# marinlauber/WaterLily

Hardware: AMD Instinct MI355X
Metric: MLUPS (cell-updates/s) per sim_step!, 3D sphere (higher is better)
Workload: dtype f32; 1 GPU; 3D sphere 512x512x512, Re=3700, f32, uniform inflow, remeasure=false (BASELINE configs[2]); layout=padded, transport=none, comm_ranks=1, scalar_allreduce=none

## Files before the change

profiles/parse_pmc.py:

```python
#!/usr/bin/env python3
import collections
import csv
import json
import os
import re
import sys

LAMBDA = {
    ("op_pcg", "k_range_red", "#1"): "pcg_init", ("op_pcg", "k_range_red", "#2"): "pcg_mult_dot",
    ("op_pcg", "k_range_red", "#3"): "pcg_update", ("op_pcg", "k_range", "#1"): "pcg_direction",
    ("op_increment", "k_range", "#1"): "increment", ("op_jacobi", "k_range", "#1"): "jacobi",
    ("op_residual", "k_range_red", "#1"): "residual", ("op_bdim2", "k_range", "#1"): "bdim",
    ("op_correct", "k_range", "#1"): "correct", ("op_div", "k_range", "#1"): "div",
}


S7 = {"op_pcg": "pcg_mult_dot", "op_increment": "increment", "op_residual": "residual", "op_smooth_fused": "smooth",
      "op_prolong_increment_fused": "prolongate"}


ROWVEC = {("op_pcg", "#1"): "pcg_init", ("op_pcg", "#2"): "pcg_update", ("op_pcg", "#3"): "pcg_direction",
          ("op_bdim2", "#1"): "bdim", ("op_scale_all", "#1"): "scale"}


def classify(name):
    if "k_convdiff3" in name:
        return "conv_diff"
    if "k_correct3" in name:
        return "correct"
    if "k_measure_fill" in name:
        return "measure_fill"
    if "k_measure_rows" in name:
        return "measure_rows"
    if "k_scale_flat" in name:
        return "scale"
    if "k_rowvec" in name:
        m = re.search(r"(op_\w+?)<", name)
        o = re.search(r"#(\d)\}", name)
        return ROWVEC.get((m.group(1), "#" + o.group(1))) if m and o else None
    if "k_stencil7" in name:
        if "ResidualDivEpi" in name:
            return "residual"
        m = re.search(r"(op_\w+?)<", name)
        return S7.get(m.group(1)) if m else None
    m = re.search(r"(k_range_red|k_range)<.*?(op_\w+?)<", name)
    o = re.search(r"#(\d)\}", name)
    if not m or not o:
        return None
    return LAMBDA.get((m.group(2), m.group(1), "#" + o.group(1)))


def collect(path, counter):
    per = collections.defaultdict(list)
    for r in csv.DictReader(open(path)):
        if r["Counter_Name"] != counter:
            continue
        k = classify(r["Kernel_Name"])
        if k:
            per[k].append(float(r["Counter_Value"]) * 1024.0)
    out, info = {}, {}
    for k, v in per.items():
        top = max(v)
        fin = [x for x in v if x > 0.25 * top]
        out[k] = sum(fin) / len(fin)
        info[k] = (len(fin), min(fin), max(fin))
    return out, info


def csrc_digest():
    import hashlib
    root = os.path.dirname(os.path.dirname(os.path.abspath(__file__)))
    h = hashlib.sha1()
    d = os.path.join(root, "waterlily_amd", "csrc")
    for f in sorted(os.listdir(d)) + [os.path.join("..", "..", "include", "wlhip.h")]:
        p = os.path.join(d, f)
# ... 34 lines not shown
```

profiles/summarize_trace.py:

```python
#!/usr/bin/env python3
import collections
import csv
import re
import sys


def short(n):
    if "k_convdiff3" in n:
        return "conv_diff(lds)"
    if "ResidualDivEpi" in n:
        rr = re.search(r"k_stencil7<\w+, \d, (\d)", n)
        return f"op_residual+div[stencil7{',R=' + rr.group(1) if rr else ''}]"
    m = re.search(r"(k_stencil7|k_rowvec|k_range_red|k_range|k_finalize|k_reduce_only|k_apply)<.*?(op_\w+?|red_\w+?)<", n)
    if m:
        lam = re.search(r"#(\d)\}", n)
        rr = re.search(r"k_stencil7<\w+, \d, (\d)", n)
        return f"{m.group(2)}{'#' + lam.group(1) if lam else ''}[{m.group(1)[2:]}{',R=' + rr.group(1) if rr else ''}]"
    if "k_pforce" in n:
        return "pforce"
    return re.sub(r"<.*", "", n)[:40]


def main():
    path = sys.argv[1]
    steps = float(sys.argv[2]) if len(sys.argv) > 2 else 1.0
    durs = collections.defaultdict(list)
    for r in csv.DictReader(open(path)):
        durs[short(r["Kernel_Name"])].append((int(r["End_Timestamp"]) - int(r["Start_Timestamp"])) / 1e3)
    rows = []
    for k, v in durs.items():
        top = max(v)
        fin = [d for d in v if top >= 60 and d > 0.25 * top]
        rest = [d for d in v if not (top >= 60 and d > 0.25 * top)]
        rows.append((k, fin, rest))
    tot_f = sum(sum(f) for _, f, _ in rows)
    tot_r = sum(sum(r) for _, _, r in rows)
    print(f"{'kernel':52s} {'finest#':>8s} {'ms':>9s} {'avg us':>8s} {'min':>7s} {'max':>7s} | {'other#':>7s} {'ms':>8s} {'avg us':>7s}   (per {steps:g} step(s))")
    for k, f, r in sorted(rows, key=lambda x: -(sum(x[1]) + sum(x[2]))):
        fa = f"{sum(f) / len(f):8.1f} {min(f):7.1f} {max(f):7.1f}" if f else f"{'':8s} {'':7s} {'':7s}"
        ra = f"{sum(r) / len(r):7.1f}" if r else f"{'':7s}"
        print(f"{k:52s} {len(f) / steps:8.1f} {sum(f) / 1e3 / steps:9.3f} {fa} | {len(r) / steps:7.1f} {sum(r) / 1e3 / steps:8.3f} {ra}")
    print(f"{'TOTAL':52s} {'':8s} {tot_f / 1e3 / steps:9.3f} {'':24s} | {'':7s} {tot_r / 1e3 / steps:8.3f}")


if __name__ == "__main__":
# ... 2 lines not shown
```

waterlily_amd/csrc/wl_api.hip:

```cpp
#include <cstdarg>
#include <cstring>
#include <memory>

#include <fcntl.h>
#include <sys/mman.h>
#include <sys/stat.h>
#include <unistd.h>

#include <rccl/rccl.h>

#include "wl_ops.h"
#include "wl_coarse.h"
#include "wl_measure.h"
#include "wl_mesh.h"
#include "wl_stats.h"
#include "wl_probe.h"
#include "wl_integrals.h"
#include "wl_surface.h"
#include "wl_iso.h"
#include "wl_render.h"

namespace wl {

struct RcclComm : Comm {
// ... 223 lines not shown
    long nband = -1;
};

template <class T> static LevelT<T> lvl(const wl_mg *m, int l) {
    const wl_level_desc &d = m->lev[l];
    LevelT<T> o;
    o.g = mkG(&d.g);
    o.L = (T *)d.L; o.D = (T *)d.D; o.iD = (T *)d.iD; o.x = (T *)d.x; o.eps = (T *)d.eps; o.r = (T *)d.r; o.z = (T *)d.z;
    o.rowc = (opt(WL_OPT_ROW_CONST_L) && l < (int)m->rowc.size()) ? (const T *)m->rowc[l].get() : nullptr;
    return o;
}

template <class T, int D> static int mg_update(wl_mg *m, const unsigned char *dirty = nullptr) {
    {
        LevelT<T> p = lvl<T>(m, 0);
        WL_TRY((op_set_diag<T, D>(p.g, p.D, p.iD, p.L, dirty)));
        WL_TRY((halo_exchange<T>(p.g, p.iD, 1, 1)));
        if (D == 3 && m->rowc[0].get()) WL_TRY((op_lrow<T>(p.g, p.L, p.iD, (T *)m->rowc[0].get(), dirty)));
    }
    for (int l = 1; l < m->nlev; ++l) {
        LevelT<T> a = lvl<T>(m, l), b = lvl<T>(m, l - 1);
        WL_TRY((op_restrictL<T, D>(a.g, a.L, b.g, b.L, m->permask)));
        WL_TRY((coarse_L_finish<T, D>(a.g, a.L, b.g, m->permask)));
        WL_TRY((op_set_diag<T, D>(a.g, a.D, a.iD, a.L)));
        WL_TRY((halo_exchange<T>(a.g, a.iD, 1, 1)));
        if (D == 3 && m->rowc[l].get()) WL_TRY((op_lrow<T>(a.g, a.L, a.iD, (T *)m->rowc[l].get())));
    }
    return 0;
}

template <class T, int D> static int mg_vcycle(wl_mg *m, int l, int *pcg_np = nullptr) {
    LevelT<T> fine = lvl<T>(m, l), coarse = lvl<T>(m, l + 1);
    const bool fused = (m->permask == 0) && opt(WL_OPT_SMOOTH_FUSED);
    if (fused) WL_TRY((op_smooth_fused<T, D>(fine, fine.eps)));
    else WL_TRY((op_jacobi<T, D>(fine, 1, m->permask)));
    const bool zero_in_restrict = (m->permask == 0) && !coarse.g.dist && !fine.g.dist;
    WL_TRY((op_restrict<T, D>(coarse.g, coarse.r, fine.g, fused ? fine.eps : fine.r, zero_in_restrict ? coarse.x : (T *)nullptr)));
    if (ctx().comm && ctx().comm->size > 1 && fine.g.dist && !coarse.g.dist) {
        const int nzl = (fine.g.nzg - 2) / ctx().comm->size / 2;
        WL_TRY(ctx().comm->allgather(coarse.r + coarse.g.s[2], (size_t)nzl * coarse.g.s[2] * sizeof(T)));
    }
    if (!zero_in_restrict) {
        Prof p(WL_K_MISC, coarse.g.cells());
        WL_HIP(hipMemsetAsync(coarse.x, 0, (size_t)span(coarse.g) * sizeof(T), ctx().stream));
    }
    const long tail_cells = coarse_tail_cells();
    bool tail = tail_cells && fused && !coarse.g.dist && coarse.g.interior_cells() <= tail_cells && (m->nlev - (l + 1)) <= CV_MAXLEV;
    if (tail) {
        CoarseArgs<T> ca;
        ca.nlev = m->nlev - (l + 1);
        for (int q = 0; q < ca.nlev; ++q) {
            ca.lev[q] = lvl<T>(m, l + 1 + q);
            if (ca.lev[q].g.dist) tail = false;
        }
        if (tail) {
            Prof p(WL_K_SMOOTH, coarse.g.cells());
            if (opt(WL_OPT_COARSE_PCG_RESIDENT)) hipLaunchKernelGGL((k_coarse_vcycle<T, D, true>), dim3(1), dim3(CV_THREADS), 0, ctx().stream, ca);
            else hipLaunchKernelGGL((k_coarse_vcycle<T, D, false>), dim3(1), dim3(CV_THREADS), 0, ctx().stream, ca);
            WL_HIP(hipGetLastError());
        }
    }
    if (!tail) {
        int pre = -1;
        if (l + 2 < m->nlev) WL_TRY((mg_vcycle<T, D>(m, l + 1, pcg_np ? &pre : nullptr)));
        WL_TRY((op_pcg<T, D>(coarse, 6, m->permask, m->sc.partials.get(), m->sc.st.get(), false, pre)));
    }
    if (pcg_np) *pcg_np = -1;
    if (fused) return op_prolong_increment_fused<T, D>(fine, fine.eps, coarse.g, coarse.x, m->sc.partials.get(), pcg_np);
    WL_TRY((op_prolongate<T, D>(fine.g, fine.eps, coarse.g, coarse.x)));
    return op_increment<T, D>(fine, m->permask);
}

template <class T, int D> static int mg_Linf(wl_mg *m, int l) {
    LevelT<T> p = lvl<T>(m, l);
    const T *r = p.r;
    return op_reduce<T, D>(p.g, WL_K_DOT, RED_MAX, 0.0, [=] __device__(long I) { const double v = (double)r[I]; return v < 0 ? -v : v; },
                           m->sc.partials.get(), m->sc.st.get(), 1, true);
}
template <class T, int D> static int mg_log_row(wl_mg *m, int n, bool have_r2) {
    if (!have_r2) WL_TRY((op_L2<T, D>(lvl<T>(m, 0), m->sc.partials.get(), m->sc.st.get(), false)));
    WL_TRY((mg_Linf<T, D>(m, 0)));
    WL_TRY(m->sc.fetch());
    m->log.push_back((double)n); m->log.push_back(m->sc.hst.get()->out[1]); m->log.push_back(m->sc.hst.get()->r2);
    return 0;
}
template <class T, int D> static int mg_solve(wl_mg *m, double tol, int itmx, int *n_iter, const T *divu = nullptr, const G *gu = nullptr,
                                              bool halo_begun = false) {
    LevelT<T> p = lvl<T>(m, 0);
    WL_TRY((op_residual<T, D>(p, m->permask, m->sc.partials.get(), m->sc.st.get(), divu, gu, halo_begun)));
    int n = 0;
    if (m->log_on) WL_TRY((mg_log_row<T, D>(m, 0, false)));
    while (n < itmx) {
        int pre = -1;
        if (m->nlev > 1) WL_TRY((mg_vcycle<T, D>(m, 0, &pre)));
        WL_TRY((op_pcg<T, D>(p, 6, m->permask, m->sc.partials.get(), m->sc.st.get(), true, pre, true)));
        WL_TRY((op_L2<T, D>(p, m->sc.partials.get(), m->sc.st.get(), true)));
        WL_TRY(m->sc.fetch());
        ++n;
        const double r2 = m->sc.hst.get()->r2;
        if (m->log_on) WL_TRY((mg_log_row<T, D>(m, n, true)));
        if (r2 < tol) break;
// ... 22 lines not shown
    bool begun = false;
    if (fused_div && g.dist) {
        if (!head_done) WL_TRY((op_scale_all<T, D>(g, p.x, dts, false, dbl)));
        if (exchange_u) { WL_TRY((halo_begin2<T>(g, uv, D, 1, p.g, p.x, 1, 1))); begun = true; }
    } else if (exchange_u && D == 3 && g.dist && overlap_on() && R.hi[2] - R.lo[2] + 1 >= 2) {
        WL_TRY((halo_begin<T>(g, uv, D, 1)));
        int rc = head_done ? 0 : op_scale_all<T, D>(g, p.x, dts, false, dbl);
        if (!rc) rc = op_div<T, D>(g, p.z, (const T *)uv, R.lo[2], R.hi[2] - 1);
        WL_TRY(halo_end());
        if (rc) return rc;
        WL_TRY((op_div<T, D>(g, p.z, (const T *)uv, R.hi[2], R.hi[2])));
    } else {
        if (exchange_u) WL_TRY((halo_exchange<T>(g, uv, D, 1)));
        if (!fused_div) WL_TRY((op_div<T, D>(g, p.z, (const T *)uv)));
        if (!head_done) WL_TRY((op_scale_all<T, D>(g, p.x, dts, false, dbl)));
    }
    WL_TRY((mg_solve<T, D>(b, 1e-4, 32, n_iter, fused_div ? (const T *)uv : nullptr, &g, begun)));
    WL_TRY((op_correct<T, D>(g, uv, p.L, p.x, p.rowc, xbc, xdone)));
    return op_scale_all<T, D>(g, p.x, dts, true, dbl, tail_then);
}

template <class T, int D>
static int flow_mom_step(wl_flow *a, wl_mg *b, double dt, const double *U, const double *gp, const double *gc,
                         double *dt_next, int *n2) {
    const wl_flow_desc &d = a->d;
    const G g = mkG(&d.g);
    T *u = (T *)d.u, *u0 = (T *)d.u0, *f = (T *)d.f, *V = (T *)d.V, *mu0 = (T *)d.mu0, *mu1 = (T *)d.mu1;
    const XBc<T> xbc{(D == 3 && d.perdir_mask == 0 && opt(WL_OPT_BC_FUSED) && opt(WL_OPT_XGHOST_IN_KERNEL)) ? 1 : 0, d.exitBC ? 1 : 0, (T)U[0]};
    bool xd = false;
    bool turns = false;
    if constexpr (D == 3)
        turns = opt(WL_OPT_BDIM_IN_CONVDIFF) && opt(WL_OPT_BDIM_ROWFLAGS) && a->rowfree && a->busy.get() && d.perdir_mask == 0 && !d.exitBC && conv_diff_tiled<D>(g, 0);
    T *const up = turns ? u0 : u;
    const CdFin<T> fin1{up, a->rowfree, xbc.on, (T)U[0]}, fin2{u, a->rowfree, xbc.on, (T)U[0]};
    (void)fin1; (void)fin2;
    if (turns) {
        if constexpr (D == 3) {
            WL_TRY((op_conv_diff<T, D, true, false, 1>(g, f, u, d.nu, 0, u, V, dt, gp, gp != nullptr, nullptr, false, &fin1)));
            WL_TRY((op_bdim2_busy<T, 1>(g, up, up, f, V, mu0, mu1, a->busy.get(), a->nbusy, a->nbusy_lo, a->nbusy_hi, xbc, a->segfree())));
            xd = xbc.on != 0;
        }
    } else {
        WL_TRY((op_conv_diff<T, D, true, true>(g, f, u, d.nu, d.perdir_mask, nullptr, V, dt, gp, gp != nullptr, u0)));
        if (d.perdir_mask != 0) WL_TRY((op_sigma_ghosts<T, D>(g, (T *)d.sigma, u, d.nu, d.perdir_mask)));
        WL_TRY((op_bdim2<T, D, 1>(g, u, f, V, mu0, mu1, a->rowfree, a->busy.get(), a->nbusy, true, &xbc, &xd, a->segfree())));
    }
    WL_TRY((op_bc_vec<T, D>(g, up, U, d.exitBC, d.perdir_mask, xd)));
    if (d.exitBC) WL_TRY((op_exit_bc<T, D>(g, up, u0, U, dt, a->sc.partials.get(), a->sc.st.get())));
    const ScaleOp corr_head = project_scale<T>(dt, 0.5);
    const bool chain = opt(WL_OPT_SCALE_CHAIN) != 0;
    WL_TRY((flow_project<T, D>(a, b, dt, 1.0, &n2[0], true, false, chain ? &corr_head : nullptr, &xbc, &xd, up)));
    WL_TRY((op_bc_vec<T, D>(g, up, U, d.exitBC, d.perdir_mask, xd)));
    if (turns) {
        if constexpr (D == 3) {
            WL_TRY((op_conv_diff<T, D, true, false, 2>(g, f, up, d.nu, 0, u, V, dt, gc, gc != nullptr, nullptr, true, &fin2)));
            WL_TRY((op_sigma_ghosts<T, D>(g, (T *)d.sigma, up, d.nu, 0)));
            WL_TRY((op_bdim2_busy<T, 2>(g, u, up, f, V, mu0, mu1, a->busy.get(), a->nbusy, a->nbusy_lo, a->nbusy_hi, xbc, a->segfree())));
            xd = xbc.on != 0;
        }
    } else {
        WL_TRY((op_conv_diff<T, D, true>(g, f, u, d.nu, d.perdir_mask, u0, V, dt, gc, gc != nullptr, nullptr, true)));
        WL_TRY((op_sigma_ghosts<T, D>(g, (T *)d.sigma, u, d.nu, d.perdir_mask)));
        WL_TRY((op_bdim2<T, D, 2>(g, u, f, V, mu0, mu1, a->rowfree, a->busy.get(), a->nbusy, true, &xbc, &xd, a->segfree())));
    }
    WL_TRY((op_bc_vec<T, D>(g, u, U, d.exitBC, d.perdir_mask, xd)));
    WL_TRY((flow_project<T, D>(a, b, dt, 0.5, &n2[1], true, chain, nullptr, &xbc, &xd)));
    WL_TRY((op_bc_vec<T, D>(g, u, U, d.exitBC, d.perdir_mask, xd)));
// ... 76 lines not shown
            const double m = (double)(T)(pv * (rx * nds[b * 2 + 1] - ry * nds[b * 2]));
            acc[0] += m; acc[1] += m;
        }
    }
    block_red<3>(acc, RED_SUM);
    if (threadIdx.x == 0)
        for (int c = 0; c < 3; ++c) partials[(long)c * gridDim.x + blockIdx.x] = acc[c];
}
template <class T>
__global__ __launch_bounds__(256) void k_pforce(const T *p, const int64_t *idx, const double *nds, int64_t nband, int D,
                                                 double *partials) {
    double acc[3] = {0, 0, 0};
    for (int64_t b = (int64_t)blockIdx.x * 256 + threadIdx.x; b < nband; b += (int64_t)gridDim.x * 256) {
        const double pv = (double)p[idx[b]];
        for (int c = 0; c < D; ++c) acc[c] += (double)(T)(pv * nds[b * D + c]);
    }
    block_red<3>(acc, RED_SUM);
    if (threadIdx.x == 0)
        for (int c = 0; c < 3; ++c) partials[(long)c * gridDim.x + blockIdx.x] = acc[c];
}
static int flow_compact_busy(wl_flow *a, const G &g, int D) {
    a->rowfree = a->rowbuf.get();
    const size_t nrows = (size_t)g.n[1] * (size_t)(D > 2 ? g.n[2] : 1);
    std::vector<unsigned char> fl(nrows);
    WL_HIP(hipMemcpyAsync(fl.data(), a->rowbuf.get(), nrows, hipMemcpyDeviceToHost, ctx().stream));
    WL_HIP(hipStreamSynchronize(ctx().stream));
    const Range R = r_inside(g);
    std::vector<int> list;
    for (int k = R.lo[2]; k <= R.hi[2]; ++k)
        for (int j = 1; j <= g.n[1] - 2; ++j)
            if (!fl[(size_t)j + (size_t)g.n[1] * k]) list.push_back(j + g.n[1] * k);
    const size_t nl = list.size();
    WL_TRY(a->busy.reserve(nl ? nl : 1, nl ? nl * 2 + 64 : 64));
    if (!list.empty()) WL_HIP(hipMemcpyAsync(a->busy.get(), list.data(), list.size() * sizeof(int), hipMemcpyHostToDevice, ctx().stream));
    WL_HIP(hipStreamSynchronize(ctx().stream));
    a->nbusy = (int)list.size();
    a->nbusy_lo = a->nbusy_hi = 0;
    if (D > 2 && R.hi[2] > R.lo[2])
        for (int row : list) { a->nbusy_lo += (row / g.n[1] == R.lo[2]); a->nbusy_hi += (row / g.n[1] == R.hi[2]); }
    else
        a->nbusy_lo = a->nbusy;
    return 0;
}
template <class T, int D> static int flow_update(wl_flow *a) {
    const G g = mkG(&a->d.g);
    WL_TRY((op_rowflags<T, D>(g, (const T *)a->d.V, (const T *)a->d.mu0, (const T *)a->d.mu1, a->rowbuf.get(), a->d.perdir_mask, D == 3 ? a->segbuf.get() : nullptr)));
    a->seg_valid = (D == 3 && a->segbuf.get() != nullptr);
    a->prev_valid = false;
    return flow_compact_busy(a, g, D);
}
static BodyDev body_dev(const wl_body_desc *bodies) {
    BodyDev o;
    o.n = bodies[0].count > 0 ? bodies[0].count : 1;
    for (int l = 0; l < o.n; ++l) {
        const wl_body_desc *b = bodies + l;
        LeafDev &d = o.leaf[l];
        d.family = b->family; d.ident = b->identity_map != 0; d.op = b->op;
        for (int q = 0; q < 8; ++q) d.p[q] = b->p[q];
        for (int q = 0; q < 9; ++q) { d.A[q] = b->A[q]; d.dA[q] = b->dA[q]; d.Ainv[q] = b->Ainv[q]; }
        for (int q = 0; q < 3; ++q) { d.b[q] = b->b[q]; d.db[q] = b->db[q]; }
    }
    for (int l = o.n; l < WL_BODY_MAXLEAF; ++l) o.leaf[l] = o.leaf[0];
    return o;
}
static int measure_alloc(wl_flow *a, size_t nrows) {
    WL_TRY(a->rowcount.reserve(nrows));
// ... 1095 lines not shown
```

waterlily_amd/csrc/wl_common.h:

```cpp
#pragma once
#include <hip/hip_runtime.h>

#include <cfloat>
#include <cstdint>
#include <cstdio>
#include <string>
#include <vector>

#include <cstdlib>

#include "../../include/wlhip.h"
#include "wl_buf.h"

namespace wl {

struct DevMem;
template <unsigned FLAGS> struct PinnedMem;

struct TimedEvt { hipEvent_t a, b; int64_t cells; };

struct Comm {
    int rank = 0, size = 1;
    int64_t cnt[6] = {0, 0, 0, 0, 0, 0};
    int depth = 0;
// ... 521 lines not shown
        return (int)hipGetLastError();
    }
    int rc = reduce_allreduce<NV>(partials, np, op, init, red);
    if (rc) return rc;
    hipLaunchKernelGGL((k_apply<FIN>), dim3(1), dim3(1), 0, ctx().stream, (const double *)red, fin);
    return (int)hipGetLastError();
}
template <class T> inline int halo_exchange(const G &g, T *a, int ncomp, int depth) {
    Comm *cm = ctx().comm;
    if (!g.dist || !cm || cm->size == 1) return 0;
    const size_t bytes = (size_t)depth * (size_t)g.s[2] * sizeof(T);
    const bool lo = g.zring || cm->rank > 0, hi = g.zring || cm->rank < cm->size - 1;
    const int plo = lo ? (cm->rank - 1 + cm->size) % cm->size : -1, phi = hi ? (cm->rank + 1) % cm->size : -1;
    int rc = cm->group_begin();
    if (rc) return rc;
    for (int c = 0; c < ncomp; ++c) {
        T *b = a + (long)c * g.sc;
        rc = cm->sendrecv(lo ? b + (long)g.zlo * g.s[2] : nullptr, lo ? b + (long)(g.zlo - depth) * g.s[2] : nullptr,
                          hi ? b + (long)(g.zhi - depth + 1) * g.s[2] : nullptr,
                          hi ? b + (long)(g.zhi + 1) * g.s[2] : nullptr, bytes, plo, phi);
        if (rc) { (void)cm->group_end(); return rc; }
    }
    return cm->group_end();
}

inline bool overlap_on() {
    Ctx &c = ctx();
    if (c.overlap < 0) {
        const char *e = getenv("WL_OVERLAP");
        c.overlap = (e && e[0] == '0') ? 0 : 1;
    }
    return c.overlap == 1 && c.comm && c.comm->size > 1;
}
template <class T> inline int halo_begin2(const G &ga, T *a, int ncompa, int deptha, const G &gb, T *b, int ncompb, int depthb) {
    Ctx &c = ctx();
    if (!ga.dist || !c.comm || c.comm->size == 1) return 0;
    auto both = [&]() -> int {
        int rc = c.comm->group_begin();
        if (rc) return rc;
        rc = halo_exchange<T>(ga, a, ncompa, deptha);
        if (!rc && b) rc = halo_exchange<T>(gb, b, ncompb, depthb);
        const int rce = c.comm->group_end();
        return rc ? rc : rce;
    };
    if (!overlap_on()) return both();
    if (!c.cstream) {
        WL_HIP(hipStreamCreateWithFlags(&c.cstream, hipStreamNonBlocking));
        WL_HIP(hipEventCreateWithFlags(&c.ev_prod, hipEventDisableTiming));
        WL_HIP(hipEventCreateWithFlags(&c.ev_halo, hipEventDisableTiming));
    }
    WL_HIP(hipEventRecord(c.ev_prod, c.stream));
    WL_HIP(hipStreamWaitEvent(c.cstream, c.ev_prod, 0));
    hipStream_t compute = c.stream;
    c.stream = c.cstream;
    const int rc = both();
    c.stream = compute;
    if (rc) return rc;
    WL_HIP(hipEventRecord(c.ev_halo, c.cstream));
    c.halo_pending = true;
    return 0;
}
template <class T> inline int halo_begin(const G &g, T *a, int ncomp, int depth) {
    return halo_begin2<T>(g, a, ncomp, depth, g, (T *)nullptr, 0, 0);
}
inline int halo_end() {
    Ctx &c = ctx();
// ... 118 lines not shown
```

waterlily_amd/csrc/wl_convdiff.h:

```cpp
#pragma once
#include <type_traits>

#include "wl_common.h"

namespace wl {

constexpr int CD_BX = 64, CD_BY = 4, CD_H = 2;
constexpr int CD_W = CD_BX + 2 * CD_H;
constexpr int CD_R = CD_BY + 2 * CD_H;
constexpr int CD_HALO = CD_W * CD_R - CD_BX * CD_BY;

template <class T, bool GEN = true>
__device__ __forceinline__ double cd_flux(T fm2, T fm1, T f0, T fp1, double uf, T nu, bool lowbnd, bool topbnd) {
    if (!GEN) { lowbnd = false; topbnd = false; }
    const bool neg = uf < 0;
    const bool up = topbnd ? !neg : (uf > 0);
    const T q = quick<T>(up ? fm2 : fp1, up ? fm1 : f0, up ? f0 : fm1);
    const double cen = (double)((T)(f0 + fm1) * (T)0.5);
    const bool central = (lowbnd && uf > 0) || (topbnd && neg);
    const double flux = uf * (central ? cen : (double)q);
    const T nud = nu * (T)(f0 - fm1);
    return flux - (double)nud;
}
template <class T, bool GEN = true> __device__ __forceinline__ T cd_add(T r, double F, bool bnd) {
    if (!GEN) return r + (T)F;
    return bnd ? (T)((double)r + F) : r + (T)F;
}
template <class T, bool GEN = true> __device__ __forceinline__ T cd_sub(T r, double F, bool bnd) {
    if (!GEN) return r - (T)F;
    return bnd ? (T)((double)r - F) : r - (T)F;
}

template <class T> struct CdFin { T *unew; const unsigned char *rowfree; int xon; T U0; };
template <class T, int FIN> __device__ __forceinline__ T cd_fin(T uold, T fv) {
    const T tmp = fv + (T)0;
    if (FIN == 1) return tmp;
    const T un = uold + tmp;
    return un * (T)0.5;
}
template <class T, bool XEDGE = true> __device__ __forceinline__ void cd_fin_store(const CdFin<T> &fn, long o, int c, int i, int n0, T val) {
    if (XEDGE && fn.xon) {
        if (i == 1) { if (c == 0) val = fn.U0; fn.unew[o - 1] = val; }
        if (i == n0 - 2) fn.unew[o + 1] = (c == 0) ? fn.U0 : val;
    }
    fn.unew[o] = val;
}

constexpr int CD_NSEG = 4;
struct CdSeg { int b0, nblk, tpp, clen, ty0, ntile, zlo, zhi; };
struct CdSegs { int n; CdSeg s[CD_NSEG]; };
template <class T, bool FUSE, bool COPY, int FIN>
__global__ __launch_bounds__(CD_BX *CD_BY) void k_convdiff3(G g, T *__restrict__ r, const T *__restrict__ u, T nu,
                                                           const T *u0, T *u0out, const T *__restrict__ V, T dt,
                                                           double a0, double a1, double a2, bool has_acc, int ntx,
                                                           CdSegs segs, CdFin<T> fn) {
    __shared__ T sm[3][3][CD_R][CD_W];
    const int tx = threadIdx.x & (CD_BX - 1), ty = threadIdx.x / CD_BX;
    CdSeg sg = segs.s[0];
#pragma unroll
    for (int q = 1; q < CD_NSEG; ++q)
        if (q < segs.n && (int)blockIdx.x >= segs.s[q].b0) sg = segs.s[q];
    const int nblk = sg.nblk, tpp = sg.tpp, clen = sg.clen, ty0 = sg.ty0, ntile = sg.ntile, zlo = sg.zlo, zhi = sg.zhi;
    const int b = (int)blockIdx.x - sg.b0;
    const int lb = (nblk & 7) ? b : (b & 7) * (nblk >> 3) + (b >> 3);
    const int ch = lb / tpp, pt = lb - ch * tpp;
    const int i0 = 1 + CD_BX * (pt % ntx), j0 = CD_BY * (ty0 + pt / ntx);
// ... 190 lines not shown
        if (h < NHALO) {
            int row, cl;
            if (h < 4 * CD_W) { const int rr = h / CD_W; row = rr < 2 ? rr : rr + BY; cl = h - rr * CD_W; }
            else { const int qq = h - 4 * CD_W; row = CD_H + (qq >> 2); const int c4 = qq & 3; cl = c4 < 2 ? c4 : c4 + CD_BX; }
            const int gx = min(max(i0 - CD_H + cl, 0), n0 - 1), gy = min(max(j0 - CD_H + row, 0), n1 - 1);
            hl[nh] = row * CD_W + cl;
            hg[nh] = (long)gx + g.s[1] * (long)gy;
            ++nh;
        }
    }
    const int own_l = (ty + CD_H) * CD_W + tx + CD_H;
    auto clampk = [n2](int k) { return min(max(k, 0), n2 - 1); };
    auto SM = [&](int slot, int c) -> T * { return &sm[slot][c][0][0]; };

    T W[3][4];
#pragma unroll
    for (int c = 0; c < 3; ++c)
#pragma unroll
        for (int q = 0; q < 4; ++q) W[c][q] = u[col + sz * clampk(k0 - 2 + q) + sc * c];
#pragma unroll
    for (int pl = 0; pl < 2; ++pl) {
        const int kk = clampk(k0 - 1 + pl);
        const int slot = (k0 - 1 + pl + 3) % 3;
#pragma unroll
        for (int c = 0; c < 3; ++c) {
            SM(slot, c)[own_l] = W[c][1 + pl];
#pragma unroll
            for (int q = 0; q < 2; ++q) if (q < nh) SM(slot, c)[hl[q]] = u[hg[q] + sz * kk + sc * c];
        }
    }
    __syncthreads();

    T cfx[3] = {0, 0, 0}, cfy[3] = {0, 0, 0}, cfz[3] = {0, 0, 0}, cu0[3] = {0, 0, 0}, cV[3] = {0, 0, 0};
    bool carry = false, cfin = false;
    const unsigned char *ffp = fn.rowfree + j;
    unsigned char ffl = 0;
    if (FIN) ffl = ffp[(long)n1 * k0];

    for (int k = k0; k <= k1; ++k) {
        const bool own = k < k1;
        const int par = k & 1;
        T nxt[3], hv[2][3], e0[3] = {0, 0, 0}, eV[3] = {0, 0, 0};
        const int kn = clampk(k + 2), kh = clampk(k + 1);
        bool fin = false;
        if (FIN) { fin = own && ffl != 0; ffl = ffp[(long)n1 * kh]; }
#pragma unroll
        for (int c = 0; c < 3; ++c) {
            nxt[c] = u[col + sz * kn + sc * c];
#pragma unroll
            for (int q = 0; q < 2; ++q) if (q < nh) hv[q][c] = u[hg[q] + sz * kh + sc * c];
            if (FUSE && own) {
                e0[c] = (COPY || FIN == 1) ? W[c][2] : u0[col + sz * k + sc * c];
                eV[c] = V[(fin ? 0L : col + sz * k) + sc * c];
            }
            if (COPY && own && active) u0out[col + sz * k + sc * c] = W[c][2];
        }
        const int s1 = (k + 3) % 3, s0 = (k + 2) % 3;
        T fx[3] = {0, 0, 0}, fy[3] = {0, 0, 0}, fz[3];
#pragma unroll
        for (int c = 0; c < 3; ++c) {
            double ufz;
            if (c == 0) ufz = (double)((T)(W[2][2] + SM(s1, 2)[own_l - 1]) * (T)0.5);
            else if (c == 1) ufz = (double)((T)(W[2][2] + SM(s1, 2)[own_l - CD_W]) * (T)0.5);
            else ufz = (double)((T)(W[2][2] + W[2][1]) * (T)0.5);
            fz[c] = (T)cd_flux<T, false>(W[c][0], W[c][1], W[c][2], W[c][3], ufz, nu, false, false);
        }
        if (carry) {
            const int pp = par ^ 1;
#pragma unroll
            for (int c = 0; c < 3; ++c) {
                T fxh = lane_dn1(cfx[c]);
                const double xe = xedge[pp][c][ty];
                const bool lastc = (i + 1 == ie);
                if (lastc) fxh = (T)xe;
                const T fyh = (ty < BY - 1) ? fyb[pp][c][ty + 1][tx] : yedge[pp][c][tx];
                T v = (T)0 + cfx[c];
                v = (GENX && xtop && lastc) ? (T)((double)v - xe) : v - fxh;
                v = v + cfy[c];
                v = v - fyh;
                v = v + cfz[c];
                v = v - fz[c];
                if (active) {
                    const long o = col + sz * (k - 1) + sc * c;
                    if (FUSE) {
                        if (has_acc) v = (T)((double)v + (c == 0 ? a0 : (c == 1 ? a1 : a2)));
                        const T fv = (cu0[c] + dt * v) - ((FIN && cfin) ? (T)0 : cV[c]);
                        r[o] = fv;
                        if (FIN) { if (cfin) cd_fin_store<T, GENX>(fn, o, c, i, n0, cd_fin<T, FIN>(W[c][1], fv)); }
                    } else {
                        r[o] = v;
                    }
                }
            }
        }
        if (own) {
#pragma unroll
            for (int c = 0; c < 3; ++c) {
                const T *P = SM(s1, c) + own_l;
                const T xm2 = P[-2], xm1 = P[-1], x0 = W[c][2], xp1 = P[1];
                const T *PX = SM(s1, 0) + own_l;
                double ufl;
                if (c == 0) ufl = (double)((T)(PX[0] + PX[-1]) * (T)0.5);
                else if (c == 1) ufl = (double)((T)(PX[0] + PX[-CD_W]) * (T)0.5);
                else ufl = (double)((T)(PX[0] + W[0][1]) * (T)0.5);
                fx[c] = (T)cd_flux<T, GENX>(xm2, xm1, x0, xp1, ufl, nu, xlow && (i == 1), false);
                const T ym2 = P[-2 * CD_W], ym1 = P[-CD_W], yp1 = P[CD_W];
                const T *PY = SM(s1, 1) + own_l;
                double vfl;
                if (c == 0) vfl = (double)((T)(PY[0] + PY[-1]) * (T)0.5);
                else if (c == 1) vfl = (double)((T)(PY[0] + PY[-CD_W]) * (T)0.5);
                else vfl = (double)((T)(PY[0] + W[1][1]) * (T)0.5);
                fy[c] = (T)cd_flux<T, false>(ym2, ym1, x0, yp1, vfl, nu, false, false);
                fyb[par][c][ty][tx] = fy[c];
            }
            if (ty < 3) {
                const int c = ty;
                const int el = (BY + CD_H) * CD_W + tx + CD_H;
                const T *P = SM(s1, c) + el;
                const T *PY = SM(s1, 1) + el;
                double vf;
                if (c == 0) vf = (double)((T)(PY[0] + PY[-1]) * (T)0.5);
                else if (c == 1) vf = (double)((T)(PY[0] + PY[-CD_W]) * (T)0.5);
                else vf = (double)((T)(PY[0] + SM(s0, 1)[el]) * (T)0.5);
                yedge[par][c][tx] = (T)cd_flux<T, false>(P[-2 * CD_W], P[-CD_W], P[0], P[CD_W], vf, nu, false, false);
            } else if (ty == 3 && tx < 3 * BY) {
                const int rr = tx / 3, c = tx - 3 * rr;
                const int xl = (rr + CD_H) * CD_W + (ie - i0) + CD_H;
                const T *P = SM(s1, c) + xl;
                const T *PX = SM(s1, 0) + xl;
                double uf;
                if (c == 0) uf = (double)((T)(PX[0] + PX[-1]) * (T)0.5);
                else if (c == 1) uf = (double)((T)(PX[0] + PX[-CD_W]) * (T)0.5);
                else uf = (double)((T)(PX[0] + SM(s0, 0)[xl]) * (T)0.5);
                const T fp1 = (ie + 1 <= n0 - 1) ? P[1] : P[0];
                xedge[par][c][rr] = cd_flux<T, GENX>(P[-2], P[-1], P[0], fp1, uf, nu, false, xtop);
            }
        }
        carry = own; cfin = fin;
#pragma unroll
        for (int c = 0; c < 3; ++c) { cfx[c] = fx[c]; cfy[c] = fy[c]; cfz[c] = fz[c]; cu0[c] = e0[c]; cV[c] = eV[c]; }
        const int s2 = (k + 4) % 3;
#pragma unroll
        for (int c = 0; c < 3; ++c) {
            W[c][0] = W[c][1]; W[c][1] = W[c][2]; W[c][2] = W[c][3]; W[c][3] = nxt[c];
            SM(s2, c)[own_l] = W[c][2];
#pragma unroll
            for (int q = 0; q < 2; ++q) if (q < nh) SM(s2, c)[hl[q]] = hv[q][c];
        }
        __syncthreads();
    }
}
template <class T, bool FUSE, bool COPY, int BY, int FIN>
__global__ __launch_bounds__(CD_BX *BY) void k_convdiff3s(G g, T *__restrict__ r, const T *__restrict__ u, T nu, const T *u0, T *u0out,
                                                         const T *__restrict__ V, T dt, double a0, double a1, double a2, bool has_acc,
                                                         int ntx, int tpp, int nblk, int clen, int jbase, int klo, int khi, int ntile, int rev,
                                                         CdFin<T> fn) {
    extern __shared__ __attribute__((aligned(16))) unsigned char cds_raw[];
    CdsShared<T, BY> &S_ = *reinterpret_cast<CdsShared<T, BY> *>(cds_raw);
    const int b = blockIdx.x;
    int lb, pslot;
    tile_of(b, nblk, rev, lb, pslot);
    (void)pslot;
    const int ch = lb / tpp, pt = lb - ch * tpp;
    const int n0 = g.n[0], n1 = g.n[1];
    const int i0 = 1 + CD_BX * (pt % ntx), j0 = jbase + BY * (pt / ntx);
    const int k0 = klo + ch * clen, k1 = min(khi + 1, k0 + clen);
    if (k0 > khi || pt >= ntile || j0 + BY - 1 > n1 - 3 || i0 > n0 - 2) return;
    const int ie = min(i0 + CD_BX, n0 - 1);
    if (i0 == 1 || ie == n0 - 1) convdiff3s_tile<T, FUSE, COPY, true, BY, FIN>(S_, g, r, u, nu, u0, u0out, V, dt, a0, a1, a2, has_acc, i0, j0, ie, k0, k1, fn);
    else convdiff3s_tile<T, FUSE, COPY, false, BY, FIN>(S_, g, r, u, nu, u0, u0out, V, dt, a0, a1, a2, has_acc, i0, j0, ie, k0, k1, fn);
}
// ... 86 lines not shown
```

waterlily_amd/csrc/wl_ops.h:

```cpp
#pragma once
#include "wl_common.h"
#include "wl_convdiff.h"
#include "wl_stencil7.h"

namespace wl {

struct State {
    double rho, alpha, beta;
    double shift;
    double r2;
    double out[4];
    double red[4];
    int active;
    int do_shift;
    int nupd;
    int r2_valid;
    int xpend;
    PcgS slots[2];
};

template <class T> struct LevelT {
    G g;
    T *L, *D, *iD, *x, *eps, *r, *z;
    const T *rowc = nullptr;
// ... 1024 lines not shown
            const int rcv = launch_stencil7_halo<T, 0>(WL_K_INCREMENT, p.g, p.eps, SrcArray<T>{p.eps}, p.L, p.rowc, p.r, p.x,
                [=] __device__(long o, int, int, int, const VA &ae, const VA &ec, const VA &r0, const VA &x0, const auto &, double *, const Pre &) {
                VA rv = r0, xv = x0;
_Pragma("unroll")
                for (int v = 0; v < VA::V; ++v) { rv.v[v] = rv.v[v] - ae.v[v]; xv.v[v] = xv.v[v] + ec.v[v]; }
                rv.store(q.r + o);
                xv.store(q.x + o);
            }, nullptr, nullptr);
            if (rcv >= 0) return rcv;
        }
    }
    if (!exchanged) WL_TRY((halo_exchange<T>(p.g, p.eps, 1, 1)));
    return launch_range(WL_K_INCREMENT, r_inside(p.g), [=] __device__(int i, int j, int k) {
        const long I = q.g.at(i, j, k);
        q.r[I] = q.r[I] - mult1r<T, D>(q.g, q.L, q.eps, I);
        q.x[I] = q.x[I] + q.eps[I];
    });
}

template <class T, int D>
int op_jacobi(const LevelT<T> &p, int it, int permask) {
    const LevelT<T> q = p;
    for (int n = 0; n < it; ++n) {
        WL_TRY(launch_range(WL_K_JACOBI, r_inside(p.g), [=] __device__(int i, int j, int k) {
            const long I = q.g.at(i, j, k);
            q.eps[I] = q.r[I] * q.iD[I];
        }));
        WL_TRY((op_increment<T, D>(p, permask)));
    }
    return 0;
}

template <class T, int D>
int op_smooth_fused(const LevelT<T> &p, T *rout) {
    const LevelT<T> q = p;
    bool exchanged = false;
    if constexpr (D == 3) {
        if (stencil7_ok<T>(p.g)) {
            using VA = VecA<T>;
            exchanged = true;
            const int rcv = launch_stencil7_halo<T, 0>(WL_K_SMOOTH, p.g, p.r, SrcJacobi<T>{p.r, p.iD, p.g.n[0]}, p.L, p.rowc,
                p.r, p.x, [=] __device__(long o, int, int, int, const VA &ae, const VA &ec, const VA &r0, const VA &x0, const auto &, double *, const Pre &) {
                    VA rv = r0, xv = x0;
_Pragma("unroll")
                    for (int v = 0; v < VA::V; ++v) { rv.v[v] = rv.v[v] - ae.v[v]; xv.v[v] = xv.v[v] + ec.v[v]; }
                    rv.store(rout + o);
                    xv.store(q.x + o);
                }, nullptr, nullptr);
            if (rcv >= 0) return rcv;
        }
    }
    if (!exchanged) WL_TRY((halo_exchange<T>(p.g, p.r, 1, 1)));
    return launch_range(WL_K_SMOOTH, r_inside(p.g), [=] __device__(int i, int j, int k) {
        const long I = q.g.at(i, j, k);
        T lo[D], hi[D];
_Pragma("unroll")
        for (int d = 0; d < D; ++d) { lo[d] = q.L[I + (long)d * q.g.sc]; hi[d] = q.L[I + q.g.s[d] + (long)d * q.g.sc]; }
        T dg = 0;
_Pragma("unroll")
        for (int d = 0; d < D; ++d) dg -= (lo[d] + hi[d]);
        const T e0 = q.r[I] * q.iD[I];
        T s = e0 * dg;
_Pragma("unroll")
        for (int d = 0; d < D; ++d) {
            const long sd = q.g.s[d];
            s += (q.r[I - sd] * q.iD[I - sd]) * lo[d] + (q.r[I + sd] * q.iD[I + sd]) * hi[d];
        }
        rout[I] = q.r[I] - s;
        q.x[I] = q.x[I] + e0;
    });
}
template <class T, int D>
int op_prolong_increment_fused(const LevelT<T> &p, const T *rin, const G &gc, const T *cx, double *partials = nullptr,
                               int *pcg_np = nullptr) {
    WL_TRY((halo_exchange<T>(gc, const_cast<T *>(cx), 1, 1)));
    const LevelT<T> q = p;
    const G C = gc;
    if (pcg_np) *pcg_np = -1;
    if constexpr (D == 3) {
        if (stencil7_ok<T>(p.g)) {
            using VA = VecA<T>;
            const SrcProlong<T> src{cx, C, p.g.n[0], p.g.n[1], p.g.nzg, p.g.kz0};
            if (pcg_np && partials && opt(WL_OPT_PCG_START_FUSED) && opt(WL_OPT_PCG_RECOMPUTE_PRECOND) && opt(WL_OPT_PCG_VEC)) {
                T *e0 = p.eps;
                const int tpp = (((p.g.n[0] - 2 + 64 * VA::V - 1) / (64 * VA::V)) * ((p.g.n[1] - 2 + 3) / 4) + 7) / 8 * 8;
                Gate gcap;
                if (tpp <= WL_PCG_PARTIALS) gcap.zcap = WL_PCG_PARTIALS / tpp;
                int np = 0;
                const int rcv = launch_stencil7<T, 1>(WL_K_PROLONG, p.g, src, p.L, p.rowc, rin, p.x,
                    [=] __device__(long o, int i, int, int, const VA &ae, const VA &ec, const VA &r0, const VA &x0, const auto &rk, double *acc, const Pre &) {
                        VA rv = r0, xv = x0;
                        const VA id = row_iD<T>(rk, q.iD, o, i, q.g.n[0]);
_Pragma("unroll")
                        for (int v = 0; v < VA::V; ++v) { rv.v[v] = rv.v[v] - ae.v[v]; xv.v[v] = xv.v[v] + ec.v[v]; }
                        rv.store(q.r + o);
                        xv.store(q.x + o);
                        VA ev;
_Pragma("unroll")
                        for (int v = 0; v < VA::V; ++v) { ev.v[v] = rv.v[v] * id.v[v]; acc[0] += (double)rv.v[v] * (double)ev.v[v]; }
                        ev.store(e0 + o);
                    }, partials, &np, gcap);
                if (rcv > 0) return rcv;
                if (rcv == 0) { *pcg_np = np; return 0; }
            }
            const int rcv = launch_stencil7<T, 0>(WL_K_PROLONG, p.g, src, p.L, p.rowc, rin, p.x,
                [=] __device__(long o, int, int, int, const VA &ae, const VA &ec, const VA &r0, const VA &x0, const auto &, double *, const Pre &) {
                    VA rv = r0, xv = x0;
_Pragma("unroll")
                    for (int v = 0; v < VA::V; ++v) { rv.v[v] = rv.v[v] - ae.v[v]; xv.v[v] = xv.v[v] + ec.v[v]; }
                    rv.store(q.r + o);
                    xv.store(q.x + o);
                }, nullptr, nullptr);
            if (rcv >= 0) return rcv;
        }
    }
    return launch_range(WL_K_PROLONG, r_inside(p.g), [=] __device__(int i, int j, int k) {
        const long I = q.g.at(i, j, k);
        const int gi[3] = {i, j, D > 2 ? q.g.kg(k) : 0};
        const int ng[3] = {q.g.n[0], q.g.n[1], q.g.nzg};
        auto epsat = [&](int d, int off) -> T {
            int f[3] = {gi[0], gi[1], gi[2]};
            f[d] += off;
            if (f[d] < 1 || f[d] > ng[d] - 2) return (T)0;
            return cx[C.at((f[0] + 1) / 2, (f[1] + 1) / 2, D > 2 ? (f[2] + 1) / 2 - C.kz0 : 0)];
        };
        T lo[D], hi[D];
_Pragma("unroll")
        for (int d = 0; d < D; ++d) { lo[d] = q.L[I + (long)d * q.g.sc]; hi[d] = q.L[I + q.g.s[d] + (long)d * q.g.sc]; }
        T dg = 0;
_Pragma("unroll")
        for (int d = 0; d < D; ++d) dg -= (lo[d] + hi[d]);
        const T e0 = epsat(0, 0);
        T s = e0 * dg;
_Pragma("unroll")
        for (int d = 0; d < D; ++d) s += epsat(d, -1) * lo[d] + epsat(d, +1) * hi[d];
        q.r[I] = rin[I] - s;
        q.x[I] = q.x[I] + e0;
    });
}

enum class PcgForm { FINALIZE, IN_KERNEL, SLAB };
template <class T> struct PcgDots {
    PcgForm form;
    State *st;
    double *partials;
    bool dist, xdef, want_r2;
    T eps10;
    int f32, zcap;
    double *P0, *PA, *PB;
    int cur = 0;
    PcgDots(PcgForm f, State *st_, double *partials_, bool dist_, bool xdef_, bool want_r2_, T eps10_, int zcap_)
        : form(f), st(st_), partials(partials_), dist(dist_), xdef(xdef_), want_r2(want_r2_), eps10(eps10_), f32(sizeof(T) == 4), zcap(zcap_) {
        const bool own = f != PcgForm::FINALIZE;
        P0 = partials; PA = own ? partials + WL_MAXB : partials; PB = own ? partials + 2 * WL_MAXB : partials;
    }
    Gate base() const { Gate g; g.eps10 = (double)eps10; g.f32 = f32; g.zcap = zcap; return g; }
    int ready(const double *&part, int &n) const {
        if (form != PcgForm::SLAB) return 0;
        Prof pr(WL_K_SCALAR, 0);
        WL_TRY((reduce_allreduce<1>(part, n, (int)RED_SUM, 0.0, st->red)));
        part = st->red;
        n = 1;
        return 0;
    }
    int after_init(int np) const {
        if (form != PcgForm::FINALIZE) return 0;
        State *s = st;
        const T e10 = eps10;
        return launch_finalize<1>(dist, partials, np, RED_SUM, 0.0, st->red, [=] __device__(const double *v) {
            const T rho = (T)v[0];
// ... 440 lines not shown
```

Measured before the change: 5701 MLUPS.

## Defer Jacobi x update into prolongation and skip dead predictor writes

The fused multigrid smoother no longer reads and writes x. The owed Jacobi correction (r*iD) is instead applied inside the fused prolong-increment kernel, through a new epilogue that loads r, x and rin together. This removes one full read and write of x per V-cycle level, at the cost of an extra r load in the prolongation. Separately, conv-diff skips storing the predictor into r for rows flagged as fully free with no busy neighbours. Both behaviours are on by default and can be masked through the WL_LEAN environment variable.

```diff
diff --git a/profiles/parse_pmc.py b/profiles/parse_pmc.py
--- a/profiles/parse_pmc.py
+++ b/profiles/parse_pmc.py
@@ -41,6 +41,8 @@
     if "k_stencil7" in name:
         if "ResidualDivEpi" in name:
             return "residual"
+        if "ProlongOwedEpi" in name:
+            return "prolongate"
         m = re.search(r"(op_\w+?)<", name)
         return S7.get(m.group(1)) if m else None
     m = re.search(r"(k_range_red|k_range)<.*?(op_\w+?)<", name)
diff --git a/profiles/summarize_trace.py b/profiles/summarize_trace.py
--- a/profiles/summarize_trace.py
+++ b/profiles/summarize_trace.py
@@ -11,6 +11,9 @@
     if "ResidualDivEpi" in n:
         rr = re.search(r"k_stencil7<\w+, \d, (\d)", n)
         return f"op_residual+div[stencil7{',R=' + rr.group(1) if rr else ''}]"
+    if "ProlongOwedEpi" in n:
+        rr = re.search(r"k_stencil7<\w+, \d, (\d)", n)
+        return f"op_prolong_increment_fused+owed[stencil7{',R=' + rr.group(1) if rr else ''}]"
     m = re.search(r"(k_stencil7|k_rowvec|k_range_red|k_range|k_finalize|k_reduce_only|k_apply)<.*?(op_\w+?|red_\w+?)<", n)
     if m:
         lam = re.search(r"#(\d)\}", n)
diff --git a/waterlily_amd/csrc/wl_api.hip b/waterlily_amd/csrc/wl_api.hip
--- a/waterlily_amd/csrc/wl_api.hip
+++ b/waterlily_amd/csrc/wl_api.hip
@@ -279,7 +279,8 @@
 template <class T, int D> static int mg_vcycle(wl_mg *m, int l, int *pcg_np = nullptr) {
     LevelT<T> fine = lvl<T>(m, l), coarse = lvl<T>(m, l + 1);
     const bool fused = (m->permask == 0) && opt(WL_OPT_SMOOTH_FUSED);
-    if (fused) WL_TRY((op_smooth_fused<T, D>(fine, fine.eps)));
+    const bool owed = fused && lean_on(WL_LEAN_SMOOTH_X);
+    if (fused) WL_TRY((op_smooth_fused<T, D>(fine, fine.eps, owed)));
     else WL_TRY((op_jacobi<T, D>(fine, 1, m->permask)));
     const bool zero_in_restrict = (m->permask == 0) && !coarse.g.dist && !fine.g.dist;
     WL_TRY((op_restrict<T, D>(coarse.g, coarse.r, fine.g, fused ? fine.eps : fine.r, zero_in_restrict ? coarse.x : (T *)nullptr)));
@@ -313,7 +314,7 @@
         WL_TRY((op_pcg<T, D>(coarse, 6, m->permask, m->sc.partials.get(), m->sc.st.get(), false, pre)));
     }
     if (pcg_np) *pcg_np = -1;
-    if (fused) return op_prolong_increment_fused<T, D>(fine, fine.eps, coarse.g, coarse.x, m->sc.partials.get(), pcg_np);
+    if (fused) return op_prolong_increment_fused<T, D>(fine, fine.eps, coarse.g, coarse.x, m->sc.partials.get(), pcg_np, owed);
     WL_TRY((op_prolongate<T, D>(fine.g, fine.eps, coarse.g, coarse.x)));
     return op_increment<T, D>(fine, m->permask);
 }
@@ -402,7 +403,7 @@
     if constexpr (D == 3)
         turns = opt(WL_OPT_BDIM_IN_CONVDIFF) && opt(WL_OPT_BDIM_ROWFLAGS) && a->rowfree && a->busy.get() && d.perdir_mask == 0 && !d.exitBC && conv_diff_tiled<D>(g, 0);
     T *const up = turns ? u0 : u;
-    const CdFin<T> fin1{up, a->rowfree, xbc.on, (T)U[0]}, fin2{u, a->rowfree, xbc.on, (T)U[0]};
+    const CdFin<T> fin1{up, a->rowfree, xbc.on, (T)U[0], lean_on(WL_LEAN_PRED_F) ? 1 : 0}, fin2{u, a->rowfree, xbc.on, (T)U[0], 0};
     (void)fin1; (void)fin2;
     if (turns) {
         if constexpr (D == 3) {
@@ -545,6 +546,18 @@
             if (!fl[(size_t)j + (size_t)g.n[1] * k]) list.push_back(j + g.n[1] * k);
     const size_t nl = list.size();
     WL_TRY(a->busy.reserve(nl ? nl : 1, nl ? nl * 2 + 64 : 64));
+    {
+        const long n1 = g.n[1], n2 = D > 2 ? g.n[2] : 1;
+        auto busy_at = [&](long j, long k) { return j >= 0 && j < n1 && k >= 0 && k < n2 && !(fl[(size_t)(j + n1 * k)] & 1); };
+        bool any = false;
+        for (int k = R.lo[2] + (g.dist ? 1 : 0); k <= R.hi[2] - (g.dist ? 1 : 0); ++k)
+            for (int j = 1; j <= g.n[1] - 2; ++j)
+                if ((fl[(size_t)j + (size_t)n1 * k] & 1) && !busy_at(j - 1, k) && !busy_at(j + 1, k) && !busy_at(j, k - 1) && !busy_at(j, k + 1)) {
+                    fl[(size_t)j + (size_t)n1 * k] |= 2;
+                    any = true;
+                }
+        if (any) WL_HIP(hipMemcpyAsync(a->rowbuf.get(), fl.data(), nrows, hipMemcpyHostToDevice, ctx().stream));
+    }
     if (!list.empty()) WL_HIP(hipMemcpyAsync(a->busy.get(), list.data(), list.size() * sizeof(int), hipMemcpyHostToDevice, ctx().stream));
     WL_HIP(hipStreamSynchronize(ctx().stream));
     a->nbusy = (int)list.size();
diff --git a/waterlily_amd/csrc/wl_common.h b/waterlily_amd/csrc/wl_common.h
--- a/waterlily_amd/csrc/wl_common.h
+++ b/waterlily_amd/csrc/wl_common.h
@@ -577,6 +577,11 @@
     }
     return c.overlap == 1 && c.comm && c.comm->size > 1;
 }
+enum { WL_LEAN_SMOOTH_X = 1, WL_LEAN_PRED_F = 2 };
+inline bool lean_on(int bit) {
+    const char *e = getenv("WL_LEAN");
+    return ((e && e[0]) ? atoi(e) : ~0) & bit;
+}
 template <class T> inline int halo_begin2(const G &ga, T *a, int ncompa, int deptha, const G &gb, T *b, int ncompb, int depthb) {
     Ctx &c = ctx();
     if (!ga.dist || !c.comm || c.comm->size == 1) return 0;
diff --git a/waterlily_amd/csrc/wl_convdiff.h b/waterlily_amd/csrc/wl_convdiff.h
--- a/waterlily_amd/csrc/wl_convdiff.h
+++ b/waterlily_amd/csrc/wl_convdiff.h
@@ -31,7 +31,7 @@
     return bnd ? (T)((double)r - F) : r - (T)F;
 }
 
-template <class T> struct CdFin { T *unew; const unsigned char *rowfree; int xon; T U0; };
+template <class T> struct CdFin { T *unew; const unsigned char *rowfree; int xon; T U0; int skipf = 0; };
 template <class T, int FIN> __device__ __forceinline__ T cd_fin(T uold, T fv) {
     const T tmp = fv + (T)0;
     if (FIN == 1) return tmp;
@@ -288,7 +288,7 @@
     __syncthreads();
 
     T cfx[3] = {0, 0, 0}, cfy[3] = {0, 0, 0}, cfz[3] = {0, 0, 0}, cu0[3] = {0, 0, 0}, cV[3] = {0, 0, 0};
-    bool carry = false, cfin = false;
+    bool carry = false, cfin = false, cdead = false;
     const unsigned char *ffp = fn.rowfree + j;
     unsigned char ffl = 0;
     if (FIN) ffl = ffp[(long)n1 * k0];
@@ -298,8 +298,8 @@
         const int par = k & 1;
         T nxt[3], hv[2][3], e0[3] = {0, 0, 0}, eV[3] = {0, 0, 0};
         const int kn = clampk(k + 2), kh = clampk(k + 1);
-        bool fin = false;
-        if (FIN) { fin = own && ffl != 0; ffl = ffp[(long)n1 * kh]; }
+        bool fin = false, dead = false;
+        if (FIN) { fin = own && ffl != 0; dead = FIN == 1 && fin && fn.skipf && (ffl & 2); ffl = ffp[(long)n1 * kh]; }
 #pragma unroll
         for (int c = 0; c < 3; ++c) {
             nxt[c] = u[col + sz * kn + sc * c];
@@ -341,7 +341,7 @@
                     if (FUSE) {
                         if (has_acc) v = (T)((double)v + (c == 0 ? a0 : (c == 1 ? a1 : a2)));
                         const T fv = (cu0[c] + dt * v) - ((FIN && cfin) ? (T)0 : cV[c]);
-                        r[o] = fv;
+                        if (!(FIN == 1 && cdead)) r[o] = fv;
                         if (FIN) { if (cfin) cd_fin_store<T, GENX>(fn, o, c, i, n0, cd_fin<T, FIN>(W[c][1], fv)); }
                     } else {
                         r[o] = v;
@@ -392,7 +392,7 @@
                 xedge[par][c][rr] = cd_flux<T, GENX>(P[-2], P[-1], P[0], fp1, uf, nu, false, xtop);
             }
         }
-        carry = own; cfin = fin;
+        carry = own; cfin = fin; cdead = dead;
 #pragma unroll
         for (int c = 0; c < 3; ++c) { cfx[c] = fx[c]; cfy[c] = fy[c]; cfz[c] = fz[c]; cu0[c] = e0[c]; cV[c] = eV[c]; }
         const int s2 = (k + 4) % 3;
diff --git a/waterlily_amd/csrc/wl_ops.h b/waterlily_amd/csrc/wl_ops.h
--- a/waterlily_amd/csrc/wl_ops.h
+++ b/waterlily_amd/csrc/wl_ops.h
@@ -1080,21 +1080,31 @@
 }
 
 template <class T, int D>
-int op_smooth_fused(const LevelT<T> &p, T *rout) {
+int op_smooth_fused(const LevelT<T> &p, T *rout, bool defer_x = false) {
     const LevelT<T> q = p;
     bool exchanged = false;
     if constexpr (D == 3) {
         if (stencil7_ok<T>(p.g)) {
             using VA = VecA<T>;
             exchanged = true;
-            const int rcv = launch_stencil7_halo<T, 0>(WL_K_SMOOTH, p.g, p.r, SrcJacobi<T>{p.r, p.iD, p.g.n[0]}, p.L, p.rowc,
-                p.r, p.x, [=] __device__(long o, int, int, int, const VA &ae, const VA &ec, const VA &r0, const VA &x0, const auto &, double *, const Pre &) {
-                    VA rv = r0, xv = x0;
-_Pragma("unroll")
-                    for (int v = 0; v < VA::V; ++v) { rv.v[v] = rv.v[v] - ae.v[v]; xv.v[v] = xv.v[v] + ec.v[v]; }
-                    rv.store(rout + o);
-                    xv.store(q.x + o);
-                }, nullptr, nullptr);
+            int rcv;
+            if (defer_x)
+                rcv = launch_stencil7_halo<T, 0>(WL_K_SMOOTH, p.g, p.r, SrcJacobi<T>{p.r, p.iD, p.g.n[0]}, p.L, p.rowc, p.r, (const T *)nullptr,
+                    [=] __device__(long o, int, int, int, const VA &ae, const VA &, const VA &r0, const VA &, const auto &, double *, const Pre &) {
+                        VA rv = r0;
+_Pragma("unroll")
+                        for (int v = 0; v < VA::V; ++v) rv.v[v] = rv.v[v] - ae.v[v];
+                        rv.store(rout + o);
+                    }, nullptr, nullptr);
+            else
+                rcv = launch_stencil7_halo<T, 0>(WL_K_SMOOTH, p.g, p.r, SrcJacobi<T>{p.r, p.iD, p.g.n[0]}, p.L, p.rowc, p.r, p.x,
+                    [=] __device__(long o, int, int, int, const VA &ae, const VA &ec, const VA &r0, const VA &x0, const auto &, double *, const Pre &) {
+                        VA rv = r0, xv = x0;
+_Pragma("unroll")
+                        for (int v = 0; v < VA::V; ++v) { rv.v[v] = rv.v[v] - ae.v[v]; xv.v[v] = xv.v[v] + ec.v[v]; }
+                        rv.store(rout + o);
+                        xv.store(q.x + o);
+                    }, nullptr, nullptr);
             if (rcv >= 0) return rcv;
         }
     }
@@ -1115,12 +1125,48 @@
             s += (q.r[I - sd] * q.iD[I - sd]) * lo[d] + (q.r[I + sd] * q.iD[I + sd]) * hi[d];
         }
         rout[I] = q.r[I] - s;
-        q.x[I] = q.x[I] + e0;
+        if (!defer_x) q.x[I] = q.x[I] + e0;
     });
 }
+template <class T, bool START> struct ProlongOwedEpi {
+    static constexpr bool HAS_LD = true;
+    using VA = VecA<T>;
+    struct Dat { VA r1, x0, rj; };
+    struct Carry {};
+    const T *rin, *iD;
+    T *r, *x, *e0;
+    int n0;
+    __device__ __forceinline__ Dat ld(long o, int, int, int) const {
+        Dat d;
+        d.r1 = VA::load(rin + o); d.x0 = VA::load(x + o); d.rj = VA::load(r + o);
+        return d;
+    }
+    __device__ __forceinline__ Carry first(long, int, int) const { return Carry{}; }
+    __device__ __forceinline__ Carry next(const Dat &) const { return Carry{}; }
+    template <class RKT>
+    __device__ __forceinline__ void operator()(long o, int i, int, int, const VA &ae, const VA &ec, const Dat &d, const Carry &, const RKT &rk,
+                                               double *acc, const Pre &) const {
+        const VA id = row_iD<T>(rk, iD, o, i, n0);
+        VA rv, xv;
+_Pragma("unroll")
+        for (int v = 0; v < VA::V; ++v) {
+            const T ej = d.rj.v[v] * id.v[v];
+            rv.v[v] = d.r1.v[v] - ae.v[v];
+            xv.v[v] = (d.x0.v[v] + ej) + ec.v[v];
+        }
+        rv.store(r + o);
+        xv.store(x + o);
+        if (START) {
+            VA ev;
+_Pragma("unroll")
+            for (int v = 0; v < VA::V; ++v) { ev.v[v] = rv.v[v] * id.v[v]; acc[0] += (double)rv.v[v] * (double)ev.v[v]; }
+            ev.store(e0 + o);
+        }
+    }
+};
 template <class T, int D>
 int op_prolong_increment_fused(const LevelT<T> &p, const T *rin, const G &gc, const T *cx, double *partials = nullptr,
-                               int *pcg_np = nullptr) {
+                               int *pcg_np = nullptr, bool owed_jacobi = false) {
     WL_TRY((halo_exchange<T>(gc, const_cast<T *>(cx), 1, 1)));
     const LevelT<T> q = p;
     const G C = gc;
@@ -1129,13 +1175,16 @@
         if (stencil7_ok<T>(p.g)) {
             using VA = VecA<T>;
             const SrcProlong<T> src{cx, C, p.g.n[0], p.g.n[1], p.g.nzg, p.g.kz0};
+            const T *const none = nullptr;
             if (pcg_np && partials && opt(WL_OPT_PCG_START_FUSED) && opt(WL_OPT_PCG_RECOMPUTE_PRECOND) && opt(WL_OPT_PCG_VEC)) {
                 T *e0 = p.eps;
                 const int tpp = (((p.g.n[0] - 2 + 64 * VA::V - 1) / (64 * VA::V)) * ((p.g.n[1] - 2 + 3) / 4) + 7) / 8 * 8;
                 Gate gcap;
                 if (tpp <= WL_PCG_PARTIALS) gcap.zcap = WL_PCG_PARTIALS / tpp;
                 int np = 0;
-                const int rcv = launch_stencil7<T, 1>(WL_K_PROLONG, p.g, src, p.L, p.rowc, rin, p.x,
+                const int rcv = owed_jacobi ? launch_stencil7<T, 1>(WL_K_PROLONG, p.g, src, p.L, p.rowc, none, none,
+                                                                    ProlongOwedEpi<T, true>{rin, p.iD, p.r, p.x, e0, p.g.n[0]}, partials, &np, gcap)
+                                            : launch_stencil7<T, 1>(WL_K_PROLONG, p.g, src, p.L, p.rowc, rin, p.x,
                     [=] __device__(long o, int i, int, int, const VA &ae, const VA &ec, const VA &r0, const VA &x0, const auto &rk, double *acc, const Pre &) {
                         VA rv = r0, xv = x0;
                         const VA id = row_iD<T>(rk, q.iD, o, i, q.g.n[0]);
@@ -1151,7 +1200,9 @@
                 if (rcv > 0) return rcv;
                 if (rcv == 0) { *pcg_np = np; return 0; }
             }
-            const int rcv = launch_stencil7<T, 0>(WL_K_PROLONG, p.g, src, p.L, p.rowc, rin, p.x,
+            const int rcv = owed_jacobi ? launch_stencil7<T, 0>(WL_K_PROLONG, p.g, src, p.L, p.rowc, none, none,
+                                                                ProlongOwedEpi<T, false>{rin, p.iD, p.r, p.x, nullptr, p.g.n[0]}, nullptr, nullptr)
+                                        : launch_stencil7<T, 0>(WL_K_PROLONG, p.g, src, p.L, p.rowc, rin, p.x,
                 [=] __device__(long o, int, int, int, const VA &ae, const VA &ec, const VA &r0, const VA &x0, const auto &, double *, const Pre &) {
                     VA rv = r0, xv = x0;
 _Pragma("unroll")
@@ -1182,8 +1233,10 @@
         T s = e0 * dg;
 _Pragma("unroll")
         for (int d = 0; d < D; ++d) s += epsat(d, -1) * lo[d] + epsat(d, +1) * hi[d];
+        T xv = q.x[I];
+        if (owed_jacobi) xv = xv + q.r[I] * q.iD[I];
         q.r[I] = rin[I] - s;
-        q.x[I] = q.x[I] + e0;
+        q.x[I] = xv + e0;
     });
 }
 
```

Result: no change. 5778 MLUPS (median of 2 runs) (+1.3%).
